# conix-center/pointcloud_stitching

Measured on AMD Instinct MI355X. Metric: Mpoints/s stitched (8x1280x720 streams: deproject+transform+RGB+pack), higher is better.
Workload: dtype f32

## Files before the change

pointcloud_stitching_amd/csrc/pcs_capi.cpp:

```cpp

#include <algorithm>
#include <cmath>
#include <cstdarg>
#include <cstdio>
#include <cstdlib>
#include <cstring>
#include <exception>
#include <new>
#include <string>
#include <vector>

#include "pcs_host.h"

using namespace pcs_host;

namespace pcs_host {

thread_local std::string g_create_err;

int fail(pcs_ctx* c, int status, const char* fmt, ...)
{
    char buf[512];
    va_list ap;
    va_start(ap, fmt);
// ... 133 lines not shown
bool certify_no_overflow(const pcs_stream_config& s, const Certificate& c, const float* M)
{
    if (!c.fast || !(c.p2_low > 0)) return false;
    if (s.color.model != PCS_DISTORTION_NONE && coeffs_nonzero(s.color)) return false;
    const double lim = std::ldexp(1.0, 30), infl = 1.0 + std::ldexp(1.0, -18);
    for (int r = 0; r < 3; r++) {
        double a = 0;
        for (int k = 0; k < 4; k++) if (!std::isfinite(M[4 * r + k])) return false;
        a = std::fabs((double)M[4 * r]) * c.xb + std::fabs((double)M[4 * r + 1]) * c.yb + std::fabs((double)M[4 * r + 2]) * c.zb +
            std::fabs((double)M[4 * r + 3]);
        if (!(a * 1000.0 * infl < lim)) return false;
    }
    const double x = c.a_max[0] / c.p2_low * infl, y = c.a_max[1] / c.p2_low * infl;
    const double xf = x * std::fabs((double)s.color.fx) * infl + std::fabs((double)s.color.ppx) + 2.0;
    const double yf = y * std::fabs((double)s.color.fy) * infl + std::fabs((double)s.color.ppy) + 2.0;
    return xf * infl < lim && yf * infl < lim;
}

bool row_magic(uint32_t W, uint32_t H, uint32_t& magic, uint32_t& shift)
{
    magic = shift = 0;
    if (W < 2) return false;
    uint32_t l = 0;
    while ((1ull << l) < W) l++;
    const unsigned __int128 m = (((unsigned __int128)1 << (31 + l)) / W) + 1;
    if (m >> 32) return false;
    magic = (uint32_t)m; shift = l - 1;
    auto ok = [&](uint64_t i) { return (uint32_t)(((uint64_t)i * magic) >> 32) >> shift == (uint32_t)(i / W); };
    for (uint64_t r = 0; r < H; r++) {
        const uint64_t a = r * W, b = r * W + W - 1;
        if (a >= (1ull << 31)) break;
        if (!ok(a) || (b < (1ull << 31) && !ok(b))) { magic = shift = 0; return false; }
    }
    if (!ok((1ull << 31) - 1)) { magic = shift = 0; return false; }
    return true;
}

uint32_t cutoff_dmax(const pcs_stream_config& s, const StreamParams& p, const std::vector<float>& mx)
{
    if (!p.z_zero_iff_d_zero || p.ddist || !(s.depth_scale > 0.0f)) return 0;
    double mxmax = 0;
    for (float v : mx) { if (!std::isfinite(v)) return 0; mxmax = std::max(mxmax, std::fabs((double)v)); }
    if (!(1.5 * mxmax < 2.0 - 1.0 / 1024.0)) return 0;
    const volatile float scale = s.depth_scale;
    auto z_of = [&](uint32_t d) { volatile float z = scale * (float)d; return (float)z; };
    if (!(z_of(1) > 0.0f)) return 0;
    for (uint32_t d = 1; d < 65535; d += 257) if (!(z_of(d) <= z_of(d + 1))) return 0;
    uint32_t lo = 0, hi = 65535;
    if (z_of(65535) <= 1.5f) return 65535;
    while (hi - lo > 1) { const uint32_t mid = (lo + hi) / 2; if (z_of(mid) <= 1.5f) lo = mid; else hi = mid; }
    return lo;
}

inline uint32_t tiles_of(uint32_t n) { return (n + kTilePoints - 1) / kTilePoints; }

int alloc_raster_slab(pcs_ctx* c, uint8_t*& slab, std::vector<uint16_t*>& depth, std::vector<uint8_t*>& color)
{
    const auto up = [](size_t b) { return (b + 16 + 255) & ~(size_t)255; };
    size_t total = 0;
    for (int s = 0; s < c->n_streams; s++)
        total += up((size_t)c->h_params[s].n_points * sizeof(uint16_t)) + up(c->h_params[s].color_bytes);
    void* q = nullptr;
    hipError_t e = hipMalloc(&q, total + 256);
    if (e != hipSuccess) return fail(c, PCS_ERR_NOMEM, "hipMalloc(%zu) failed: %s", total, hipGetErrorString(e));
    slab = static_cast<uint8_t*>(q);
    depth.assign(c->n_streams, nullptr); color.assign(c->n_streams, nullptr);
    size_t off = 0;
    for (int s = 0; s < c->n_streams; s++) {
        depth[s] = reinterpret_cast<uint16_t*>(slab + off);
        off += up((size_t)c->h_params[s].n_points * sizeof(uint16_t));
        color[s] = slab + off;
        off += up(c->h_params[s].color_bytes);
    }
    return PCS_OK;
}

int ensure_rasters(pcs_ctx* c)
{
    if (c->s_slab) return PCS_OK;
    return alloc_raster_slab(c, c->s_slab, c->s_depth, c->s_color);
}

}

namespace pcs_host {

int ensure_voxel_ws(pcs_ctx* c, size_t need)
{
    if (need <= c->s_voxel_ws_cap && c->s_voxel_ws) return PCS_OK;
    const size_t exact = need;
    if (c->s_voxel_ws) {
        HIPCHK(c, hipStreamSynchronize(c->stream));
        need += need / 4;
    }
    c->vox_state.clean = false;
    c->vox_state.spl_leaf = 0;
    int rc = ensure(c, c->s_voxel_ws, c->s_voxel_ws_cap, need);
    if (rc == PCS_ERR_NOMEM && need != exact) rc = ensure(c, c->s_voxel_ws, c->s_voxel_ws_cap, exact);
    return rc;
}

int acquire_event_pair(pcs_ctx* c, std::pair<hipEvent_t, hipEvent_t>& pr)
{
    if (!c->ev_free.empty()) { pr = c->ev_free.back(); c->ev_free.pop_back(); return PCS_OK; }
    HIPCHK(c, hipEventCreate(&pr.first));
    HIPCHK(c, hipEventCreate(&pr.second));
// ... 33 lines not shown
            HIPCHK(c, hipMemsetAsync(c->d_error, 0, sizeof(uint32_t), c->stream));
        }
        c->compact_seq++;
        if ((c->compact_seq & 0x3FFFFFFFu) == 0) {
            HIPCHK(c, hipMemsetAsync(c->d_desc, 0, sizeof(uint64_t) * ((size_t)c->total_tiles + PCS_MAX_STREAMS), c->stream));
            c->compact_seq++;
        }
        for (int s0 = 0; single_pass && s0 < c->n_streams; s0 += kLaunchStreams) {
            const int nl = std::min(kLaunchStreams, c->n_streams - s0);
            FramePtrs fp{};
            uint32_t tiles = 0;
            int m = 1;
            for (int k = 0; k < nl; k++) {
                fp.depth[k] = d_depth[s0 + k]; fp.color[k] = d_color[s0 + k];
                tiles += tiles_of(c->h_params[s0 + k].n_points);
                m = std::min(m, c->h_params[s0 + k].cert_fast);
            }
            CompactLaunch cl{};
            cl.d_ticket = c->compact_tickets ? c->d_ticket : nullptr; cl.ticket_base = c->tickets_issued;
            cl.d_desc = c->d_desc + c->h_params[s0].tile_base;
            cl.d_stream_end = c->d_stream_end;
            cl.d_stream_desc = c->d_desc + c->total_tiles;
            cl.d_chain_in = s0 > 0 ? c->d_stream_end + (s0 - 1) : nullptr;
            cl.d_error = c->d_error; cl.gen = c->compact_seq; cl.flags = c->flags;
            cl.d_counts = d_counts ? d_counts : c->d_counts; cl.n_total = c->n_streams;
            cl.last_launch = (s0 + nl == c->n_streams) ? 1 : 0;
            HIPCHK(c, launch_fused_compact(c->d_params, s0, nl, tiles, m >= 1 ? MathSel::Cert : MathSel::Ieee, fp, cl,
                                           d_payload, c->stream));
            c->tickets_issued += tiles;
        }
        if (c->kernel_timing) {
            HIPCHK(c, hipEventRecord(ev.second, c->stream));
            c->ev_pool.push_back(ev);
        }
        return PCS_OK;
    }
    if (pred) {
        for (int s0 = 0; !d_tile_kept && s0 < c->n_streams; s0 += kLaunchStreams) {
            const int nl = std::min(kLaunchStreams, c->n_streams - s0);
            FramePtrs fp{};
            uint32_t mp = 0;
            for (int k = 0; k < nl; k++) { fp.depth[k] = d_depth[s0 + k]; fp.color[k] = d_color[s0 + k]; mp = std::max(mp, c->h_params[s0 + k].n_points); }
            HIPCHK(c, launch_fused_count(c->d_params, s0, nl, mp, c->flags, fp, c->d_tile_counts, c->stream));
        }
        HIPCHK(c, launch_scan(c->d_params, c->n_streams, c->downsample, d_tile_kept ? d_tile_kept : c->d_tile_counts, c->d_tile_prefix,
                              c->d_stream_base, d_counts ? d_counts : c->d_counts, nullptr, c->stream));
    }
    for (int s0 = 0; s0 < c->n_streams; s0 += kLaunchStreams) {
        const int nl = std::min(kLaunchStreams, c->n_streams - s0);
        FramePtrs fp{};
        uint32_t mp = 0;
        for (int k = 0; k < nl; k++) { fp.depth[k] = d_depth[s0 + k]; fp.color[k] = d_color[s0 + k]; mp = std::max(mp, c->h_params[s0 + k].n_points); }
        bool fast = true, ident = true, noovf = true;
        bool dd = false, cd = false;
        for (int k = 0; k < nl; k++) {
            const StreamParams& q = c->h_params[s0 + k];
            fast &= q.cert_fast != 0; ident &= q.ident_r != 0; noovf &= q.no_overflow != 0;
            dd |= q.ddist != 0;
            cd |= q.cdist != 0 || q.tex_half != 0;
        }
        const MathSel sel = !fast ? MathSel::Ieee
                          : noovf ? (ident ? MathSel::CertIdentRNoOvf : MathSel::CertNoOvf)
                                  : (ident ? MathSel::CertIdentR : MathSel::Cert);
        if (dense)
            HIPCHK(c, launch_fused_dense(c->d_params, s0, nl, mp, dd, cd, sel, fp, d_payload, c->stream));
        else
            HIPCHK(c, launch_fused_emit(c->d_params, s0, nl, mp, c->flags, c->downsample, sel, fp, c->d_tile_prefix,
                                        c->d_stream_base, d_payload,
                                        pred ? (d_counts ? d_counts : c->d_counts) + c->n_streams : nullptr, c->n_streams, c->stream));
    }
    if (!pred && d_counts)
        HIPCHK(c, hipMemcpyAsync(d_counts, c->d_static_counts, sizeof(int32_t) * (c->n_streams + 1),
                                 hipMemcpyDeviceToDevice, c->stream));
    if (c->kernel_timing) {
        HIPCHK(c, hipEventRecord(ev.second, c->stream));
        c->ev_pool.push_back(ev);
    }
    return PCS_OK;
}

}

namespace {

int take_compact_error(pcs_ctx* c, bool& was_set)
{
    was_set = false;
    if (!c->d_error) return PCS_OK;
    uint32_t e = 0;
    HIPCHK(c, hipMemcpyAsync(&e, c->d_error, sizeof e, hipMemcpyDeviceToHost, c->stream));
    HIPCHK(c, hipStreamSynchronize(c->stream));
    if (e) {
        was_set = true;
        c->single_pass_ok = false;
        HIPCHK(c, hipMemsetAsync(c->d_error, 0, sizeof e, c->stream));
    }
    return PCS_OK;
}

int upload_params(pcs_ctx* c)
{
    HIPCHK(c, hipMemcpy(c->d_params, c->h_params.data(), c->h_params.size() * sizeof(StreamParams), hipMemcpyHostToDevice));
    return PCS_OK;
}

}

extern "C" {

int pcs_abi_version(void) { return PCS_ABI_VERSION; }

int pcs_device_count(void)
{
    int n = 0;
    hipError_t e = hipGetDeviceCount(&n);
    if (e != hipSuccess) return 0;
    return n;
}
// ... 144 lines not shown
            for (auto& pr : seen) if (pr.first == dim) { ok = pr.second; return hipSuccess; }
            hipError_t e;
            if (!d_bad && (e = hipMalloc((void**)&d_bad, sizeof(unsigned long long))) != hipSuccess) return e;
            if ((e = hipMemsetAsync(d_bad, 0, sizeof(unsigned long long), c->stream)) != hipSuccess) return e;
            const float cf = (float)dim, rc = (float)(1.0 / (double)cf);
            if ((e = launch_verify_div_const(cf, rc, dim, d_bad, c->stream)) != hipSuccess) return e;
            unsigned long long h = 1;
            if ((e = hipMemcpyAsync(&h, d_bad, sizeof h, hipMemcpyDeviceToHost, c->stream)) != hipSuccess) return e;
            if ((e = hipStreamSynchronize(c->stream)) != hipSuccess) return e;
            ok = (h == 0);
            seen.emplace_back(dim, ok);
            return hipSuccess;
        };
        for (int s = 0; s < c->n_streams; s++) {
            StreamParams& p = c->h_params[s];
            if (!p.cert_fast) continue;
            bool okw = false, okh = false;
            CREATE_CHK(verified(p.cW, okw));
            CREATE_CHK(verified(p.cH, okh));
            if (!(okw && okh)) { p.cert_fast = 0; p.ident_r = 0; p.no_overflow = 0; }
        }
        if (d_bad) (void)hipFree(d_bad);
    }
    c->compact_path = 0;
    if (const char* e = getenv("PCS_COMPACT_PATH")) {
        if (!strcmp(e, "single")) c->compact_path = 1;
    } else if (const char* e1 = getenv("PCS_COMPACT_SINGLE_PASS")) {
        if (e1[0] == '1') c->compact_path = 1;
    }
    c->single_pass_ok = c->compact_path == 1;
    { const char* e = getenv("PCS_COMPACT_TICKETS"); c->compact_tickets = e && e[0] == '1'; }
    c->math.resize(c->n_streams);
    for (int s = 0; s < c->n_streams; s++) {
        const StreamParams& q = c->h_params[s];
        c->math[s] = q.cert_fast ? ((q.ident_r ? 2 : 1) + (q.no_overflow ? 2 : 0)) : 0;
    }
    CREATE_CHK(hipMemcpy(c->d_params, c->h_params.data(), sizeof(StreamParams) * c->n_streams, hipMemcpyHostToDevice));
    {
        const char* env = getenv("PCS_ROW_CONST");
        const bool want = !(env && env[0] == '0');
        unsigned long long* d_bad = nullptr;
        bool any = false;
        for (int s = 0; want && s < c->n_streams; s++) {
            StreamParams& p = c->h_params[s];
            const float* t = c->cfg[s].depth_to_color.translation;
            if (p.ident_r != 1 || p.ddist || p.cdist || p.tex_half || t[1] != 0.0f || t[2] != 0.0f || !p.z_zero_iff_d_zero) continue;
            if (!d_bad) CREATE_CHK(hipMalloc((void**)&d_bad, sizeof(unsigned long long)));
            CREATE_CHK(hipMemsetAsync(d_bad, 0, sizeof(unsigned long long), c->stream));
            int32_t* d_crow = reinterpret_cast<int32_t*>(const_cast<float*>(p.my) + p.H);
            CREATE_CHK(launch_certify_color_row(c->d_params, s, p.H, d_crow, d_bad, c->stream));
            unsigned long long h = 1;
            CREATE_CHK(hipMemcpyAsync(&h, d_bad, sizeof h, hipMemcpyDeviceToHost, c->stream));
            CREATE_CHK(hipStreamSynchronize(c->stream));
            if (h == 0) { p.ident_r = 2; any = true; }
        }
        if (d_bad) (void)hipFree(d_bad);
        if (any) CREATE_CHK(hipMemcpy(c->d_params, c->h_params.data(), sizeof(StreamParams) * c->n_streams, hipMemcpyHostToDevice));
    }
#undef CREATE_CHK
    } catch (const std::exception& ex) {
        const int rc = fail(nullptr, PCS_ERR_NOMEM, "pcs_create: host allocation failed (%s)", ex.what());
        pcs_destroy(c);
        return rc;
    }
    *out = c;
    return PCS_OK;
}

void pcs_destroy(pcs_ctx* c)
{
    if (!c) return;
    DeviceGuard guard(c->device);
    if (c->stream) (void)hipStreamSynchronize(c->stream);
    for (float* p : c->d_lut) if (p) (void)hipFree(p);
    if (c->s_slab) (void)hipFree(c->s_slab);
    if (c->dl_stream) (void)hipStreamSynchronize(c->dl_stream);
    for (auto& sl : c->pipe) {
        if (sl.slab) (void)hipFree(sl.slab);
        if (sl.payload) (void)hipFree(sl.payload);
        if (sl.counts) (void)hipFree(sl.counts);
        if (sl.done) (void)hipEventDestroy(sl.done);
    }
    if (c->dl_stream) (void)hipStreamDestroy(c->dl_stream);
    void* singles[] = {c->d_params, c->d_tile_counts, c->d_tile_prefix, c->d_stream_base, c->d_counts, c->s_payload,
                       c->d_ticket, c->d_desc, c->d_stream_end, c->d_error, c->d_arrive, c->d_static_counts, c->d_batch_scratch, c->s_voxel_ws, c->s_voxel_in, c->s_voxel_out,
                       c->s_vertices, c->s_texcoords, c->s_pack_counts, c->s_pack_prefix};
    for (void* p : singles) if (p) (void)hipFree(p);
    for (auto& pr : c->ev_pool) { (void)hipEventDestroy(pr.first); (void)hipEventDestroy(pr.second); }
    for (auto& pr : c->ev_free) { (void)hipEventDestroy(pr.first); (void)hipEventDestroy(pr.second); }
    if (c->ev_begin) (void)hipEventDestroy(c->ev_begin);
    if (c->ev_end) (void)hipEventDestroy(c->ev_end);
    if (c->own_stream) (void)hipStreamDestroy(c->own_stream);
    delete c;
}

int pcs_set_cam_to_world(pcs_ctx* c, int stream, const float m16[16])
{
    if (!c || !m16) return PCS_ERR_INVALID_ARG;
    if (stream < 0 || stream >= c->n_streams) return fail(c, PCS_ERR_INVALID_ARG, "stream %d out of range", stream);
    DeviceGuard guard(c->device);
    HIPCHK(c, hipStreamSynchronize(c->stream));
    std::memcpy(c->cfg[stream].cam_to_world, m16, sizeof(float) * 16);
    StreamParams& q = c->h_params[stream];
    for (int k = 0; k < 12; k++) q.M[k] = m16[k];
    q.no_overflow = (q.cert_fast && certify_no_overflow(c->cfg[stream], c->cert[stream], m16)) ? 1 : 0;
    c->math[stream] = q.cert_fast ? ((q.ident_r ? 2 : 1) + (q.no_overflow ? 2 : 0)) : 0;
    return upload_params(c);
// ... 893 lines not shown
```

pointcloud_stitching_amd/csrc/pcs_device.h:

```cpp
#pragma once

#include <hip/hip_runtime.h>
#include <stdint.h>

#include "../../include/pcs_hip.h"

namespace pcs {

constexpr int      kBlockThreads   = 256;
constexpr int      kPointsPerLane  = 8;
constexpr uint32_t kTilePoints     = kBlockThreads * kPointsPerLane;
constexpr int      kLaunchStreams  = 16;

struct alignas(16) StreamParams {
    float    M[12];
    float    R[9];
    float    t[3];
    float    depth_scale;
    float    d_ppx, d_ppy, d_fx, d_fy;
    float    c_fx, c_fy, c_ppx, c_ppy;
    float    c_w_f, c_h_f;
    float    c_wm1_f, c_hm1_f;
    float    c_rw, c_rh;
    float    dk[5];
    float    ck[5];
    int32_t  W, H;
    int32_t  cW, cH;
    int32_t  bpp, stride;
    uint32_t color_bytes;
    uint32_t n_points;
    int32_t  ddist, cdist;
    uint32_t out_base;
    uint32_t tile_base;
    uint32_t w_magic, w_shift;
    int32_t  cert_fast;
    int32_t  ident_r;
    int32_t  no_overflow;
    int32_t  z_zero_iff_d_zero;
    uint32_t cut_dmax;
    int32_t  tex_half;
    const float* mx;
    const float* my;
};

struct FramePtrs {
    const uint16_t* depth[kLaunchStreams];
    const uint8_t*  color[kLaunchStreams];
};

struct VertexPtrs {
    const float*   vertices;
    const float*   texcoords;
    const uint8_t* color;
    uint32_t       n_points;
};

constexpr int kBatchEntries = 64;
constexpr int kBatchSets    = 16;
struct BatchPtrs {
    const uint16_t* depth[kBatchEntries];
    const uint8_t*  color[kBatchEntries];
    uint8_t*        payload[kBatchSets];
};
struct BatchCounts {
    int32_t* counts[kBatchSets];
};

constexpr int kPackBatch = 16;
struct PackBatch {
    VertexPtrs v[kPackBatch];
    uint8_t*   out[kPackBatch];
    int32_t    stream[kPackBatch];
};

enum class MathSel { Ieee = 0, Cert = 1, CertIdentR = 2, CertNoOvf = 3, CertIdentRNoOvf = 4,
                     CertRowConst = 5  };

hipError_t launch_fused_dense(const StreamParams* d_params, int stream0, int n_launch, uint32_t max_points,
                              bool any_ddist, bool any_cdist, MathSel math, const FramePtrs& fp, int16_t* d_payload,
                              hipStream_t st);

hipError_t launch_fused_count(const StreamParams* d_params, int stream0, int n_launch, uint32_t max_points,
                              uint32_t flags, const FramePtrs& fp, uint32_t* d_tile_counts, hipStream_t st);
hipError_t launch_scan(const StreamParams* d_params, int n_streams, int downsample,
                       const uint32_t* d_tile_counts, uint32_t* d_tile_prefix, uint32_t* d_stream_kept,
                       int32_t* d_counts, uint32_t* d_arrive, hipStream_t st);
hipError_t launch_fused_emit(const StreamParams* d_params, int stream0, int n_launch, uint32_t max_points,
                             uint32_t flags, int downsample, MathSel math, const FramePtrs& fp,
                             const uint32_t* d_tile_prefix, const uint32_t* d_stream_kept,
                             int16_t* d_payload, int32_t* d_total_out, int n_total_streams, hipStream_t st);
struct CompactLaunch {
    unsigned long long* d_ticket;
    unsigned long long  ticket_base;
    uint64_t*           d_desc;
    uint64_t*           d_stream_desc;
    uint32_t*           d_stream_end;
    const uint32_t*     d_chain_in;
    uint32_t*           d_error;
    uint32_t            gen;
    uint32_t            flags;
    int32_t*            d_counts;
    int32_t             n_total;
    int32_t             last_launch;
};
hipError_t launch_fused_compact(const StreamParams* d_params, int stream0, int n_launch, uint32_t launch_tiles,
                                MathSel math, const FramePtrs& fp, const CompactLaunch& cl, int16_t* d_payload,
                                hipStream_t st);

hipError_t launch_fused_dense_batch(const StreamParams* d_params, int n_streams, int n_sets, uint32_t max_points,
                                    bool any_ddist, bool any_cdist, MathSel math, const BatchPtrs& bp, hipStream_t st);
hipError_t launch_compact_batch(const StreamParams* d_params, int n_streams, int n_sets, uint32_t max_points,
                                uint32_t total_tiles, uint32_t flags, MathSel math, const BatchPtrs& bp,
                                const BatchCounts& bc, uint32_t* d_tile_counts, uint32_t* d_tile_prefix,
                                uint32_t* d_stream_kept, hipStream_t st);
hipError_t launch_verify_div_const(float c, float rc, int32_t dim, unsigned long long* d_bad, hipStream_t st);
hipError_t launch_certify_color_row(const StreamParams* d_params, int stream, int rows, int32_t* d_crow, unsigned long long* d_bad, hipStream_t st);

hipError_t launch_pack_dense(const StreamParams* d_params, int stream, const VertexPtrs& vp,
                             int16_t* d_out, hipStream_t st);
hipError_t launch_pack_count(const StreamParams* d_params, int stream, const VertexPtrs& vp, uint32_t flags,
                             uint32_t* d_tile_counts, hipStream_t st);
hipError_t launch_pack_scan(uint32_t n_tiles, const uint32_t* d_tile_counts, uint32_t* d_tile_prefix,
                            int32_t* d_out_points, uint32_t* d_arrive, hipStream_t st);
hipError_t launch_pack_emit(const StreamParams* d_params, int stream, const VertexPtrs& vp, uint32_t flags,
                            const uint32_t* d_tile_prefix, int16_t* d_out, hipStream_t st);

hipError_t launch_pack_batch(const StreamParams* d_params, const PackBatch& pb, int n, uint32_t max_points, bool aligned,
                             hipStream_t st);

// ... 67 lines not shown
```

pointcloud_stitching_amd/csrc/pcs_kernels.hip:

```cpp


#include <cstddef>

#include "pcs_device.h"

#ifndef PCS_TU_VOXEL
#define PCS_TU_VOXEL 0
#endif


#ifndef EMIT_WAVES
#define EMIT_WAVES 6
#endif

namespace pcs {

namespace {

constexpr uint32_t kDenseStageBytes = kTilePoints * PCS_POINT_BYTES;
constexpr uint32_t kStageBytes      = kTilePoints * PCS_POINT_BYTES + 32;

typedef float f32x4 __attribute__((ext_vector_type(4)));
template <class T> using gptr = const __attribute__((address_space(1))) T*;
template <class T> __device__ __forceinline__ gptr<T> as_global(const T* p)
// ... 93 lines not shown
    {
        q0 = __fdiv_rn(a0, b);
        q1 = __fdiv_rn(a1, b);
    }
    static __device__ __forceinline__ float div_const(float a, float c, float ) { return __fdiv_rn(a, c); }
};

template <bool IDENT_R, bool NO_OVERFLOW = false>
struct CertMath {
    static constexpr bool kIdentR = IDENT_R;
    static constexpr bool kRowConst = false;
    static constexpr int kCvtMode = NO_OVERFLOW ? 2 : 1;
    static __device__ __forceinline__ void d2c(const StreamParams& P, float X, float Y, float Z,
                                               float& P0, float& P1, float& P2)
    {
        if (IDENT_R) {
            P0 = __fadd_rn(X, P.t[0]);
            P1 = __fadd_rn(Y, P.t[1]);
            P2 = __fadd_rn(Z, P.t[2]);
        } else {
            IeeeMath::d2c(P, X, Y, Z, P0, P1, P2);
        }
    }
    static __device__ __forceinline__ void div2(float a0, float a1, float b, float& q0, float& q1)
    {
        float y = __builtin_amdgcn_rcpf(b);
        const float e = __fmaf_rn(-b, y, 1.0f);
        y = __fmaf_rn(e, y, y);
        float q = __fmul_rn(a0, y);
        float r = __fmaf_rn(-b, q, a0);
        q = __fmaf_rn(r, y, q);
        r = __fmaf_rn(-b, q, a0);
        q0 = __fmaf_rn(r, y, q);
        q = __fmul_rn(a1, y);
        r = __fmaf_rn(-b, q, a1);
        q = __fmaf_rn(r, y, q);
        r = __fmaf_rn(-b, q, a1);
        q1 = __fmaf_rn(r, y, q);
    }
    static __device__ __forceinline__ float div_const(float a, float c, float rc)
    {
        const float q0 = __fmul_rn(a, rc);
        const float r = __fmaf_rn(-c, q0, a);
        return __fmaf_rn(r, rc, q0);
    }
};

using CertNoOvf = CertMath<false, true>;
using CertIdentNoOvf = CertMath<true, true>;

struct CertRowConst : CertMath<true, false> {
    [[maybe_unused]] static constexpr bool kRowConst = true;
};

__device__ __forceinline__ void color_coords(const StreamParams& P, float u, float v, float& xf, float& yf)
{
    xf = __fmaf_rn(u, P.c_w_f, 0.5f);
    yf = __fmaf_rn(v, P.c_h_f, 0.5f);
}

template <class Cvt>
__device__ __forceinline__ uint32_t color_fetch(const StreamParams& P, const uint8_t* __restrict__ color,
                                                int32_t xi, int32_t yi, Cvt& cv)
{
    const uint32_t idx = __umul24((uint32_t)xi, (uint32_t)P.bpp) + __umul24((uint32_t)yi, (uint32_t)P.stride);
    uint32_t shift;
    const uint32_t off = cv.window(idx, P.color_bytes - 4u, shift);
    uint32_t w;
    __builtin_memcpy(&w, color + off, 4);
    return w >> shift;
}

__device__ __forceinline__ float world_mm(const float* __restrict__ Mr, float X, float Y, float Z)
{
    float a = __fmaf_rn(X, Mr[0], Mr[3]);
    a = __fmaf_rn(Y, Mr[1], a);
    a = __fmaf_rn(Z, Mr[2], a);
    return __fmul_rn(a, 1000.0f);
}

constexpr uint32_t kLoLo = 0x05040100u, kHiLo = 0x05040302u;
__device__ __forceinline__ uint32_t perm(uint32_t hi, uint32_t lo, uint32_t sel) { return __builtin_amdgcn_perm(hi, lo, sel); }

struct Record {
    uint32_t xy;
    uint32_t zc;
    uint32_t b;
};

__device__ __forceinline__ void stage_record(uint8_t* lds, uint32_t off, const Record& r)
{
    const bool odd = (off & 2u) != 0u;
    const uint32_t yz = perm(r.zc, r.xy, kHiLo);
    const uint32_t cc = perm(r.b, r.zc, kHiLo);
    const uint32_t h_val = odd ? r.xy : r.b;
    const uint32_t a_val = odd ? yz : r.xy;
    const uint32_t b_val = odd ? cc : r.zc;
    const uint32_t h_off = odd ? off : off + 8u;
    const uint32_t a_off = odd ? off + 2u : off;
    *reinterpret_cast<uint16_t*>(lds + h_off) = (uint16_t)h_val;
    *reinterpret_cast<uint32_t*>(lds + a_off) = a_val;
    *reinterpret_cast<uint32_t*>(lds + a_off + 4u) = b_val;
}

template <class Cvt>
__device__ __forceinline__ Record make_record(const StreamParams& P, const uint8_t* __restrict__ color,
// ... 310 lines not shown
__device__ __forceinline__ void store_staged(const uint8_t* lds, uint32_t head, uint32_t nbytes, uint8_t* g)
{
    uint8_t* g0 = g - head;
    const uint32_t end = head + nbytes;
    const uint32_t first_full = (head + 15u) >> 4;
    const uint32_t last_full = end >> 4;
    typedef uint32_t u32x4 __attribute__((ext_vector_type(4)));
    for (uint32_t j = first_full + threadIdx.x; j < last_full; j += THREADS)
        __builtin_nontemporal_store(reinterpret_cast<const u32x4*>(lds)[j], reinterpret_cast<u32x4*>(g0) + j);
    const uint32_t head_end = min(first_full << 4, end);
    for (uint32_t b = head + 2u * threadIdx.x; b < head_end; b += 2u * THREADS)
        *reinterpret_cast<uint16_t*>(g0 + b) = *reinterpret_cast<const uint16_t*>(lds + b);
    if (last_full >= first_full) {
        const uint32_t tail_begin = max(last_full << 4, head_end);
        for (uint32_t b = tail_begin + 2u * threadIdx.x; b < end; b += 2u * THREADS)
            *reinterpret_cast<uint16_t*>(g0 + b) = *reinterpret_cast<const uint16_t*>(lds + b);
    }
}

template <class Src, uint32_t THREADS = kBlockThreads>
__device__ __forceinline__ void dense_tile(const StreamParams& P, const Src& src, const uint8_t* __restrict__ color,
                                           uint32_t tile0, uint32_t n, uint8_t* __restrict__ out_bytes,
                                           uint4* stage)
{
    const uint32_t i0 = tile0 + threadIdx.x * kPointsPerLane;
    PointIn p[8];
    src.load8(P, i0, n, p);

    uint32_t w[20];
    auto fill = [&](auto& cv) {
#pragma unroll
        for (int k = 0; k < 8; k += 2) {
            const Record a = make_record(P, color, p[k], cv);
            const Record b = make_record(P, color, p[k + 1], cv);
            uint32_t* o = w + (k >> 1) * 5;
            o[0] = a.xy;
            o[1] = a.zc;
            o[2] = perm(b.xy, a.b, kLoLo);
            o[3] = perm(b.zc, b.xy, kHiLo);
            o[4] = perm(b.b, b.zc, kHiLo);
        }
    };
    if (Src::Math::kCvtMode == 2) {
        FastCvt<false> fast;
        fill(fast);
        if (__builtin_expect(fast.redo(), 0)) { ExactCvt exact; fill(exact); }
    } else if (Src::Math::kCvtMode == 1) {
        FastCvt<true> fast;
        fill(fast);
        if (__builtin_expect(fast.redo(), 0)) { ExactCvt exact; fill(exact); }
    } else {
        ExactCvt exact;
        fill(exact);
    }
    uint4* mine = stage + threadIdx.x * 5;
#pragma unroll
    for (int k = 0; k < 5; k++) mine[k] = make_uint4(w[4 * k], w[4 * k + 1], w[4 * k + 2], w[4 * k + 3]);
    __syncthreads();

    const uint32_t pts = min(THREADS * kPointsPerLane, n - tile0);
    store_staged<THREADS>(reinterpret_cast<const uint8_t*>(stage), 0u, pts * PCS_POINT_BYTES,
                          out_bytes + (size_t)tile0 * PCS_POINT_BYTES);
}

template <class Src, bool PRED, bool DS1>
__device__ __forceinline__ void generic_tile(const StreamParams& P, const Src& src, const uint8_t* __restrict__ color,
                                             uint32_t tile0, uint32_t n, uint32_t flags, uint32_t ds,
                                             uint32_t g0, uint32_t out_first, uint8_t* __restrict__ payload_bytes,
                                             uint8_t* stage, uint32_t* wsum)
{
    if (DS1) ds = 1u;
    const uint32_t i0 = tile0 + threadIdx.x * kPointsPerLane;
    PointIn p[8];
    src.load8(P, i0, n, p);

    uint32_t keep, ex = 0;
    if (PRED) {
        keep = keep_mask8(p, i0, n, flags);
        uint32_t wave_total;
        ex = wave_exclusive_scan(__popc(keep), wave_total);
        if ((threadIdx.x & 63) == 63) wsum[threadIdx.x >> 6] = wave_total;
    } else {
        const uint32_t mine = (i0 < n) ? min(8u, n - i0) : 0u;
        keep = (1u << mine) - 1u;
    }

    Record rec[8];
    auto fill = [&](auto& cv) {
#pragma unroll
        for (int k = 0; k < 8; k++) rec[k] = make_record(P, color, p[k], cv);
    };
    if (Src::Math::kCvtMode == 2) {
        FastCvt<false> fast;
        fill(fast);
        if (__builtin_expect(fast.redo(), 0)) { ExactCvt exact; fill(exact); }
    } else if (Src::Math::kCvtMode == 1) {
        FastCvt<true> fast;
        fill(fast);
        if (__builtin_expect(fast.redo(), 0)) { ExactCvt exact; fill(exact); }
    } else {
        ExactCvt exact;
        fill(exact);
    }

    uint32_t lane_first, tile_kept;
    if (PRED) {
// ... 161 lines not shown

    uint8_t* gdst = payload_bytes + (size_t)q_lo * PCS_POINT_BYTES;
    const uint32_t head = (uint32_t)((uintptr_t)gdst & 15u);
    uint32_t rank = lane_first;
#pragma unroll
    for (int k = 0; k < 8; k++) {
        if ((keep >> k) & 1u) {
            stage_record(stage, head + rank * PCS_POINT_BYTES, rec[k]);
            rank++;
        }
    }
    __syncthreads();
    store_staged(stage, head, tile_kept * PCS_POINT_BYTES, gdst);
}

#endif

template <bool LEAN = false, bool IDENT_R = false>
__device__ __forceinline__ void request_constants(const StreamParams& P, const void* a, const void* b, const void* c = nullptr)
{
    static_assert(sizeof(StreamParams) == 19 * 16, "request_constants covers the struct in 19 quads");
    static_assert(offsetof(StreamParams, dk) == 39 * 4 && offsetof(StreamParams, ck) == 44 * 4 && offsetof(StreamParams, R) == 12 * 4,
                  "quads 10, 11 = dk[1..4], ck[0..3]; quads 3, 4 = R[0..7]");
    typedef uint32_t u32x4s __attribute__((ext_vector_type(4)));
    const u32x4s* q = reinterpret_cast<const u32x4s*>(&P);
    if (LEAN && IDENT_R)
        asm volatile("" :: "s"(q[0]), "s"(q[1]), "s"(q[2]), "s"(q[5]), "s"(q[6]), "s"(q[7]), "s"(q[8]), "s"(q[9]),
                           "s"(q[12]), "s"(q[13]), "s"(q[14]), "s"(q[15]), "s"(q[16]), "s"(q[17]), "s"(q[18]),
                           "s"(a), "s"(b), "s"(c));
    else if (LEAN)
        asm volatile("" :: "s"(q[0]), "s"(q[1]), "s"(q[2]), "s"(q[3]), "s"(q[4]), "s"(q[5]), "s"(q[6]), "s"(q[7]), "s"(q[8]), "s"(q[9]),
                           "s"(q[12]), "s"(q[13]), "s"(q[14]), "s"(q[15]), "s"(q[16]), "s"(q[17]), "s"(q[18]),
                           "s"(a), "s"(b), "s"(c));
    else
        asm volatile("" :: "s"(q[0]), "s"(q[1]), "s"(q[2]), "s"(q[3]), "s"(q[4]), "s"(q[5]), "s"(q[6]), "s"(q[7]), "s"(q[8]), "s"(q[9]),
                           "s"(q[10]), "s"(q[11]), "s"(q[12]), "s"(q[13]), "s"(q[14]), "s"(q[15]), "s"(q[16]), "s"(q[17]), "s"(q[18]),
                           "s"(a), "s"(b), "s"(c));
}

#if !PCS_TU_VOXEL

template <bool DDIST, bool CDIST, class Mth, uint32_t THREADS = kBlockThreads>
__global__ __launch_bounds__(THREADS, 7)
void pcs_fused_dense_kernel(const StreamParams* __restrict__ params, int stream0, FramePtrs fp,
                            uint8_t* __restrict__ payload_bytes)
{
    __shared__ uint4 stage[THREADS * kPointsPerLane * PCS_POINT_BYTES / 16];
    const int s = blockIdx.y;
    const StreamParams& P = params[stream0 + s];
    request_constants(P, fp.depth[s], fp.color[s], payload_bytes);
    const uint32_t n = P.n_points;
    const uint32_t tile0 = blockIdx.x * (THREADS * kPointsPerLane);
    if (tile0 >= n) return;
    DepthSource<DDIST, CDIST, Mth> src{fp.depth[s]};
    dense_tile<DepthSource<DDIST, CDIST, Mth>, THREADS>(P, src, fp.color[s], tile0, n, payload_bytes + (size_t)P.out_base * PCS_POINT_BYTES, stage);
}

template <bool DDIST, bool CDIST, class Mth>
__global__ __launch_bounds__(kBlockThreads, 7)
void pcs_fused_dense_batch_kernel(const StreamParams* __restrict__ params, BatchPtrs bp)
{
    __shared__ uint4 stage[kDenseStageBytes / 16];
    const int s = blockIdx.y;
    const StreamParams& P = params[s];
    const int e = blockIdx.z * gridDim.y + s;
    request_constants(P, bp.depth[e], bp.color[e], bp.payload[blockIdx.z]);
    const uint32_t n = P.n_points;
    const uint32_t tile0 = blockIdx.x * kTilePoints;
    if (tile0 >= n) return;
    DepthSource<DDIST, CDIST, Mth> src{bp.depth[e]};
    dense_tile(P, src, bp.color[e], tile0, n, bp.payload[blockIdx.z] + (size_t)P.out_base * PCS_POINT_BYTES, stage);
}

constexpr int kCountTiles = 2;
template <bool DDIST, bool CDIST>
__device__ __forceinline__ void count_tiles(const StreamParams& P, const uint16_t* __restrict__ dp, uint32_t flags,
                                            uint32_t* __restrict__ tile_counts, uint32_t (*wsum)[4])
{
    const uint32_t n = P.n_points;
    const uint32_t tile_first = blockIdx.x * kCountTiles;
    if (tile_first * kTilePoints >= n) return;
    uint32_t c[kCountTiles];
    const bool cut = (flags & PCS_FLAG_CUTOFF) != 0;
    if (P.z_zero_iff_d_zero && (!cut || P.cut_dmax != 0u)) {
        const uint32_t dmax = cut ? P.cut_dmax : 0xFFFFu;
        uint4 dv[kCountTiles];
        const bool aligned = ((uintptr_t)dp & 15) == 0 && n >= 8;
        if (aligned) {
#pragma unroll
            for (int q = 0; q < kCountTiles; q++) {
                const uint32_t i0 = (tile_first + q) * kTilePoints + threadIdx.x * kPointsPerLane;
                dv[q] = *reinterpret_cast<const uint4*>(dp + ((i0 + 8 <= n) ? i0 : 0u));
            }
        } else {
#pragma unroll
            for (int q = 0; q < kCountTiles; q++) dv[q] = make_uint4(0, 0, 0, 0);
        }
#pragma unroll
        for (int q = 0; q < kCountTiles; q++) {
            const uint32_t i0 = (tile_first + q) * kTilePoints + threadIdx.x * kPointsPerLane;
            uint32_t dw[4] = {dv[q].x, dv[q].y, dv[q].z, dv[q].w};
            if (!(aligned && i0 + 8 <= n)) {
                dw[0] = dw[1] = dw[2] = dw[3] = 0u;
                for (uint32_t k = 0; k < 8 && i0 + k < n; k++) dw[k >> 1] |= (uint32_t)dp[i0 + k] << ((k & 1u) * 16u);
            }
            uint32_t rng = 0, nz = 0;
#pragma unroll
            for (int k = 0; k < 8; k++) {
// ... 938 lines not shown
    uint32_t local = 0;
    for (uint32_t d = 1u + threadIdx.x; d < 65536u; d += 256u) local += row_of(d) != want;
    if (local) atomicAdd(bad, (unsigned long long)local);
    if (threadIdx.x == 0) crow[r] = want;
}


__global__ __launch_bounds__(256)
void pcs_verify_div_const_kernel(float c, float rc, int32_t dim, unsigned long long* __restrict__ bad)
{
    const uint64_t stride = (uint64_t)gridDim.x * blockDim.x;
    uint32_t local = 0;
    for (uint64_t bits = (uint64_t)blockIdx.x * blockDim.x + threadIdx.x; bits < (1ull << 32); bits += stride) {
        const float a = __uint_as_float((uint32_t)bits);
        const float f1 = __fmaf_rn(IeeeMath::div_const(a, c, rc), c, 0.5f);
        const float f2 = __fmaf_rn(CertMath<false>::div_const(a, c, rc), c, 0.5f);
        const int32_t i1 = min(max(cvtt_x86(f1), 0), dim - 1);
        const int32_t i2 = min(max(cvtt_x86(f2), 0), dim - 1);
        const int32_t i3 = (f2 >= 2147483648.0f) ? i2 : min(max(cvt_sat(f2), 0), dim - 1);
        local += (i1 != i2) | (i2 != i3);
    }
    if (local) atomicAdd(bad, (unsigned long long)local);
}

#endif

constexpr uint32_t kSmallThreads = 64, kSmallTilePoints = kSmallThreads * kPointsPerLane;
inline bool small_launch(uint32_t, int)
{
    const char* v = getenv("PCS_SMALL_TILES");
    return v && v[0] == '1';
}

inline dim3 tile_grid(uint32_t max_points, int n_launch)
{
    return dim3((max_points + kTilePoints - 1) / kTilePoints, (unsigned)n_launch, 1);
}

}


#if !PCS_TU_VOXEL
hipError_t launch_fused_dense(const StreamParams* d_params, int stream0, int n_launch, uint32_t max_points,
                              bool any_ddist, bool any_cdist, MathSel math, const FramePtrs& fp, int16_t* d_payload,
                              hipStream_t st)
{
    if (n_launch <= 0 || max_points == 0) return hipSuccess;
    const bool small = small_launch(max_points, n_launch);
    const dim3 grid = small ? dim3((max_points + kSmallTilePoints - 1) / kSmallTilePoints, (unsigned)n_launch, 1) : tile_grid(max_points, n_launch);
#define L(DD, CD, M) do { if (small) hipLaunchKernelGGL((pcs_fused_dense_kernel<DD, CD, M, kSmallThreads>), grid, dim3(kSmallThreads), 0, st, \
                                        d_params, stream0, fp, reinterpret_cast<uint8_t*>(d_payload)); \
                          else hipLaunchKernelGGL((pcs_fused_dense_kernel<DD, CD, M>), grid, dim3(kBlockThreads), 0, st, \
                                        d_params, stream0, fp, reinterpret_cast<uint8_t*>(d_payload)); } while (0)
    if (math != MathSel::Ieee && !any_ddist) {
        const bool ident = (math == MathSel::CertIdentR || math == MathSel::CertIdentRNoOvf);
        const bool noovf = (math == MathSel::CertNoOvf || math == MathSel::CertIdentRNoOvf) && !any_cdist;
        if (noovf)      { if (ident) L(false, false, CertIdentNoOvf); else L(false, false, CertNoOvf); }
        else if (ident) { if (any_cdist) L(false, true, CertMath<true>); else L(false, false, CertMath<true>); }
        else            { if (any_cdist) L(false, true, CertMath<false>); else L(false, false, CertMath<false>); }
    } else {
        if (any_ddist) { if (any_cdist) L(true, true, IeeeMath); else L(true, false, IeeeMath); }
        else           { if (any_cdist) L(false, true, IeeeMath); else L(false, false, IeeeMath); }
    }
#undef L
    return hipGetLastError();
}

hipError_t launch_fused_count(const StreamParams* d_params, int stream0, int n_launch, uint32_t max_points,
                              uint32_t flags, const FramePtrs& fp, uint32_t* d_tile_counts, hipStream_t st)
{
    if (n_launch <= 0 || max_points == 0) return hipSuccess;
    const uint32_t tiles = (max_points + kTilePoints - 1) / kTilePoints;
    const dim3 grid((tiles + kCountTiles - 1) / kCountTiles, (unsigned)n_launch, 1);
    hipLaunchKernelGGL((pcs_fused_count_kernel<true, false>), grid, dim3(kBlockThreads), 0, st,
                       d_params, stream0, fp, flags, d_tile_counts);
    return hipGetLastError();
}

hipError_t launch_scan(const StreamParams* d_params, int n_streams, int downsample,
                       const uint32_t* d_tile_counts, uint32_t* d_tile_prefix, uint32_t* d_stream_kept,
                       int32_t* d_counts, uint32_t* d_arrive, hipStream_t st)
{
    hipLaunchKernelGGL(pcs_scan_kernel, dim3((unsigned)n_streams), dim3(1024), 0, st, d_params, 0, n_streams, 0u,
                       (uint32_t)downsample, d_tile_counts, d_tile_prefix, d_stream_kept, d_counts, d_arrive);
    return hipGetLastError();
}

hipError_t launch_fused_emit(const StreamParams* d_params, int stream0, int n_launch, uint32_t max_points,
                             uint32_t flags, int downsample, MathSel math, const FramePtrs& fp,
                             const uint32_t* d_tile_prefix, const uint32_t* d_stream_kept,
                             int16_t* d_payload, int32_t* d_total_out, int n_total_streams, hipStream_t st)
{
    if (n_launch <= 0 || max_points == 0) return hipSuccess;
    const dim3 grid = tile_grid(max_points, n_launch);
    const bool pred = (flags & (PCS_FLAG_CUTOFF | PCS_FLAG_DROP_INVALID)) != 0;
    const bool ds1 = downsample == 1;
    uint8_t* out = reinterpret_cast<uint8_t*>(d_payload);
#define L(PR, D1, M) hipLaunchKernelGGL((pcs_fused_emit_kernel<PR, D1, M>), grid, dim3(kBlockThreads), 0, st, d_params, \
                                        stream0, fp, flags, (uint32_t)downsample, d_tile_prefix, d_stream_kept, out, \
                                        d_total_out, n_total_streams)
#define LM(M) do { if (pred) { if (ds1) L(true, true, M); else L(true, false, M); } \
                   else      { if (ds1) L(false, true, M); else L(false, false, M); } } while (0)
    const bool ident = (math == MathSel::CertIdentR || math == MathSel::CertIdentRNoOvf);
    if (math == MathSel::Ieee) LM(IeeeMath); else if (ident) LM(CertMath<true>); else LM(CertMath<false>);
#undef LM
#undef L
// ... 234 lines not shown
```

Measured before the change: 319,300.

## Stage per-wave color row windows into LDS for row-constant dense kernel

Adds a specialized dense kernel path for streams certified to have row-constant color rows and no overflow. Each wave computes the span of color bytes its points can reach, prefetches that window into LDS with global_load_lds_dwordx4, then gathers RGB from LDS instead of scattered global loads, falling back to global reads for misses. Window bounds are precomputed on the host at create time and stored after the color row table. The path uses inline asm with hand-placed waitcnts and requires 16-byte-aligned buffers, which adds fragility in exchange for removing uncoalesced color gathers.

After: 334,100 (median of 6 runs). +4.6%, better.

```diff
diff --git a/pointcloud_stitching_amd/csrc/pcs_capi.cpp b/pointcloud_stitching_amd/csrc/pcs_capi.cpp
--- a/pointcloud_stitching_amd/csrc/pcs_capi.cpp
+++ b/pointcloud_stitching_amd/csrc/pcs_capi.cpp
@@ -209,6 +209,21 @@
     return lo;
 }
 
+constexpr double kWinShiftCols = 48.0;
+void color_window_params(const StreamParams& p, float tx, int32_t out[3])
+{
+    const double a = (double)p.c_fx / p.d_fx, b = (double)p.c_ppx - (double)p.d_ppx * a + 0.5;
+    const double room = ((3072.0 - 2 * 34) / p.bpp - 512.0 * a) / 2.0 - 4.0;
+    const double shift = std::max(0.0, std::min(kWinShiftCols, room));
+    const double lo = b - 2.0 - (tx < 0.0f ? shift : 0.0), hi = b + 2.0 + (tx > 0.0f ? shift : 0.0);
+    const double kx = std::round(a * 4096.0);
+    const double reach = kx * p.W + 4096.0 * std::max(std::fabs(lo), std::fabs(hi)) + 4096.0;
+    if (!(a > 0.0) || !(reach < 2147483647.0)) { out[0] = 0; out[1] = 0; out[2] = -4096; return; }
+    out[0] = (int32_t)kx;
+    out[1] = (int32_t)std::floor(lo * 4096.0);
+    out[2] = (int32_t)std::ceil(hi * 4096.0);
+}
+
 inline uint32_t tiles_of(uint32_t n) { return (n + kTilePoints - 1) / kTilePoints; }
 
 int alloc_raster_slab(pcs_ctx* c, uint8_t*& slab, std::vector<uint16_t*>& depth, std::vector<uint8_t*>& color)
@@ -348,10 +363,12 @@
         uint32_t mp = 0;
         for (int k = 0; k < nl; k++) { fp.depth[k] = d_depth[s0 + k]; fp.color[k] = d_color[s0 + k]; mp = std::max(mp, c->h_params[s0 + k].n_points); }
         bool fast = true, ident = true, noovf = true;
+        bool rowc = true;
         bool dd = false, cd = false;
         for (int k = 0; k < nl; k++) {
             const StreamParams& q = c->h_params[s0 + k];
             fast &= q.cert_fast != 0; ident &= q.ident_r != 0; noovf &= q.no_overflow != 0;
+            rowc &= q.ident_r == 2 && (q.W & 7) == 0 && q.color_bytes >= 16;
             dd |= q.ddist != 0;
             cd |= q.cdist != 0 || q.tex_half != 0;
         }
@@ -359,7 +376,8 @@
                           : noovf ? (ident ? MathSel::CertIdentRNoOvf : MathSel::CertNoOvf)
                                   : (ident ? MathSel::CertIdentR : MathSel::Cert);
         if (dense)
-            HIPCHK(c, launch_fused_dense(c->d_params, s0, nl, mp, dd, cd, sel, fp, d_payload, c->stream));
+            HIPCHK(c, launch_fused_dense(c->d_params, s0, nl, mp, dd, cd, sel == MathSel::CertIdentRNoOvf && rowc ? MathSel::CertRowConstNoOvf : sel,
+                                         fp, d_payload, c->stream));
         else
             HIPCHK(c, launch_fused_emit(c->d_params, s0, nl, mp, c->flags, c->downsample, sel, fp, c->d_tile_prefix,
                                         c->d_stream_base, d_payload,
@@ -610,7 +628,12 @@
             unsigned long long h = 1;
             CREATE_CHK(hipMemcpyAsync(&h, d_bad, sizeof h, hipMemcpyDeviceToHost, c->stream));
             CREATE_CHK(hipStreamSynchronize(c->stream));
-            if (h == 0) { p.ident_r = 2; any = true; }
+            if (h == 0) {
+                p.ident_r = 2; any = true;
+                int32_t win[3];
+                color_window_params(p, t[0], win);
+                CREATE_CHK(hipMemcpy(d_crow + p.H, win, sizeof win, hipMemcpyHostToDevice));
+            }
         }
         if (d_bad) (void)hipFree(d_bad);
         if (any) CREATE_CHK(hipMemcpy(c->d_params, c->h_params.data(), sizeof(StreamParams) * c->n_streams, hipMemcpyHostToDevice));
diff --git a/pointcloud_stitching_amd/csrc/pcs_device.h b/pointcloud_stitching_amd/csrc/pcs_device.h
--- a/pointcloud_stitching_amd/csrc/pcs_device.h
+++ b/pointcloud_stitching_amd/csrc/pcs_device.h
@@ -74,7 +74,8 @@
 };
 
 enum class MathSel { Ieee = 0, Cert = 1, CertIdentR = 2, CertNoOvf = 3, CertIdentRNoOvf = 4,
-                     CertRowConst = 5  };
+                     CertRowConst = 5 ,
+                     CertRowConstNoOvf = 6  };
 
 hipError_t launch_fused_dense(const StreamParams* d_params, int stream0, int n_launch, uint32_t max_points,
                               bool any_ddist, bool any_cdist, MathSel math, const FramePtrs& fp, int16_t* d_payload,
diff --git a/pointcloud_stitching_amd/csrc/pcs_kernels.hip b/pointcloud_stitching_amd/csrc/pcs_kernels.hip
--- a/pointcloud_stitching_amd/csrc/pcs_kernels.hip
+++ b/pointcloud_stitching_amd/csrc/pcs_kernels.hip
@@ -169,6 +169,9 @@
 struct CertRowConst : CertMath<true, false> {
     [[maybe_unused]] static constexpr bool kRowConst = true;
 };
+struct CertRowConstNoOvf : CertMath<true, true> {
+    [[maybe_unused]] static constexpr bool kRowConst = true;
+};
 
 __device__ __forceinline__ void color_coords(const StreamParams& P, float u, float v, float& xf, float& yf)
 {
@@ -585,6 +588,159 @@
     } else {
         ExactCvt exact;
         fill(exact);
+    }
+    uint4* mine = stage + threadIdx.x * 5;
+#pragma unroll
+    for (int k = 0; k < 5; k++) mine[k] = make_uint4(w[4 * k], w[4 * k + 1], w[4 * k + 2], w[4 * k + 3]);
+    __syncthreads();
+
+    const uint32_t pts = min(THREADS * kPointsPerLane, n - tile0);
+    store_staged<THREADS>(reinterpret_cast<const uint8_t*>(stage), 0u, pts * PCS_POINT_BYTES,
+                          out_bytes + (size_t)tile0 * PCS_POINT_BYTES);
+}
+
+constexpr uint32_t kWaveStageBytes = 64u * kPointsPerLane * PCS_POINT_BYTES;
+constexpr uint32_t kWinPieces      = 3;
+constexpr uint32_t kWinBytes       = kWinPieces * 64u * 16u;
+constexpr uint32_t kWinZeroWord    = kWaveStageBytes - 16u;
+static_assert(kWinBytes + 8u <= kWinZeroWord, "the windows, the dword read past their end and the zero word fit one wave's stage");
+
+template <class T> using cptr = const __attribute__((address_space(4))) T*;
+
+__device__ __forceinline__ void color_stretch(const StreamParams& P, const int32_t (&wp)[3], int32_t crow, int32_t c0, int32_t c1,
+                                              uint32_t room, uint32_t& ws, uint32_t& len)
+{
+    const int32_t lo = min(max((c0 * wp[0] + wp[1]) >> 12, 0), P.cW - 1);
+    const int32_t hi = min(max((c1 * wp[0] + wp[2]) >> 12, 0), P.cW - 1);
+    const uint32_t row = (uint32_t)crow * (uint32_t)P.stride;
+    ws = (row + (uint32_t)lo * (uint32_t)P.bpp) & ~15u;
+    const uint32_t we = min((row + (uint32_t)hi * (uint32_t)P.bpp + 4u + 15u) & ~15u, P.color_bytes & ~15u);
+    len = min(we > ws ? we - ws : 0u, room);
+}
+
+typedef uint32_t u32x4v __attribute__((ext_vector_type(4)));
+__device__ __forceinline__ u32x4v load16_asm(const void* base, uint32_t off)
+{
+    u32x4v v;
+    asm volatile("global_load_dwordx4 %0, %1, %2" : "=v"(v) : "v"(off), "s"(base));
+    return v;
+}
+__device__ __forceinline__ uint32_t load4_asm(const void* base, uint32_t off)
+{
+    uint32_t v;
+    asm volatile("global_load_dword %0, %1, %2" : "=v"(v) : "v"(off), "s"(base));
+    return v;
+}
+__device__ __forceinline__ void window_piece(const uint8_t* color, uint32_t off, uint32_t lds)
+{
+    uint32_t keep;
+    asm volatile("s_mov_b32 %0, m0\n\ts_mov_b32 m0, %3\n\ts_nop 0\n\tglobal_load_lds_dwordx4 %1, %2\n\ts_mov_b32 m0, %0"
+                 : "=&s"(keep) : "v"(off), "s"(color), "s"(lds) : "memory");
+}
+
+template <class Mth, uint32_t THREADS = kBlockThreads>
+__device__ __forceinline__ void dense_tile_rowc(const StreamParams& P, const uint16_t* __restrict__ depth,
+                                                const uint8_t* __restrict__ color, uint32_t tile0, uint32_t n,
+                                                uint8_t* __restrict__ out_bytes, uint4* stage)
+{
+    static_assert(Mth::kRowConst && Mth::kCvtMode == 2, "the no-overflow row-constant policy");
+    const uint32_t i0 = tile0 + threadIdx.x * kPointsPerLane;
+    const uint32_t ic = min(i0, n - kPointsPerLane);
+    const uint32_t r = P.w_magic ? (__umulhi(ic, P.w_magic) >> P.w_shift) : ic / (uint32_t)P.W;
+    const uint32_t c0 = ic - r * (uint32_t)P.W;
+    u32x4v dv = load16_asm(depth, ic * 2u);
+    u32x4v ma = load16_asm(P.mx, c0 * 4u);
+    u32x4v mb = load16_asm(P.mx, c0 * 4u + 16u);
+    uint32_t myb = load4_asm(P.my, r * 4u);
+    uint32_t crow = load4_asm(P.my, ((uint32_t)P.H + r) * 4u);
+
+    const uint32_t wave = __builtin_amdgcn_readfirstlane(threadIdx.x >> 6);
+    const uint32_t iw = tile0 + wave * 64u * kPointsPerLane;
+    const uint32_t il = min(iw + 64u * kPointsPerLane, n) - 1u;
+    const uint32_t ra = __builtin_amdgcn_readfirstlane(r), rb = __builtin_amdgcn_readlane(r, 63);
+    const cptr<int32_t> tab = (cptr<int32_t>)(uintptr_t)(P.my + P.H);
+    const int32_t wp[3] = {tab[P.H], tab[P.H + 1], tab[P.H + 2]};
+    const uint32_t lrel = wave * kWaveStageBytes;
+    uint32_t wsa = 0, lena = 0, wsb = 0, lenb = 0;
+    if (iw < n) {
+        color_stretch(P, wp, tab[ra], (int32_t)(iw - ra * (uint32_t)P.W), ra == rb ? (int32_t)(il - ra * (uint32_t)P.W) : P.W - 1,
+                      kWinBytes, wsa, lena);
+        if (rb != ra) color_stretch(P, wp, tab[rb], 0, (int32_t)(il - rb * (uint32_t)P.W), kWinBytes - lena, wsb, lenb);
+    }
+    const uint32_t lane = threadIdx.x & 63u;
+    const uint32_t pieces = max((lena + lenb) >> 4, 1u), pa = lena >> 4;
+    const uint32_t lds0 = (uint32_t)(uintptr_t)(__attribute__((address_space(3))) uint8_t*)stage + lrel;
+#pragma unroll
+    for (uint32_t k = 0; k < kWinPieces; k++) {
+        const uint32_t j = min(k * 64u + lane, pieces - 1u);
+        window_piece(color, j < pa ? wsa + 16u * j : wsb + 16u * (j - pa), lds0 + k * 1024u);
+    }
+    if (lane == 0) *reinterpret_cast<uint32_t*>(reinterpret_cast<uint8_t*>(stage) + lrel + kWinZeroWord) = *(cptr<uint32_t>)(uintptr_t)color;
+
+    static_assert(kWinPieces == 3, "the wait below leaves the window's requests in flight");
+    asm volatile("s_waitcnt vmcnt(3)" : "+v"(dv), "+v"(ma), "+v"(mb), "+v"(myb), "+v"(crow));
+    PointIn p[8];
+    {
+        const uint32_t dw[4] = {dv.x, dv.y, dv.z, dv.w};
+        const uint32_t mxs[8] = {ma.x, ma.y, ma.z, ma.w, mb.x, mb.y, mb.z, mb.w};
+#pragma unroll
+        for (int k = 0; k < 8; k++) {
+            const uint32_t d = (k & 1) ? (dw[k >> 1] >> 16) : (dw[k >> 1] & 0xFFFFu);
+            p[k] = deproject_pixel_rowc<Mth>(P, d, __uint_as_float(mxs[k]), __uint_as_float(myb), (int)crow);
+        }
+    }
+    FastCvt<false> cv;
+    uint32_t xy[8], zz[8], ci[8];
+#pragma unroll
+    for (int k = 0; k < 8; k++) {
+        const float ax = world_mm(P.M + 0, p[k].X, p[k].Y, p[k].Z);
+        const float ay = world_mm(P.M + 4, p[k].X, p[k].Y, p[k].Z);
+        const float az = world_mm(P.M + 8, p[k].X, p[k].Y, p[k].Z);
+        xy[k] = perm((uint32_t)cv.cvt(ay), (uint32_t)cv.cvt(ax), kLoLo);
+        zz[k] = (uint32_t)cv.cvt(az);
+        const int32_t xi = cv.pixel(__fmaf_rn(p[k].u, P.c_w_f, 0.5f), P.cW - 1, P.c_wm1_f);
+        ci[k] = __umul24((uint32_t)xi, (uint32_t)P.bpp) + __umul24((uint32_t)__float_as_int(p[k].v), (uint32_t)P.stride);
+    }
+    const bool in_a = r == ra;
+    const uint32_t ws = in_a ? wsa : wsb, len = in_a ? lena : lenb;
+    const uint32_t wn = len > 3u ? len - 3u : 0u;
+    const uint32_t lb = lrel + (in_a ? 0u : lena), lz = lrel + kWinZeroWord;
+    asm volatile("s_waitcnt vmcnt(0)" : "+v"(ci[0]), "+v"(ci[1]), "+v"(ci[2]), "+v"(ci[3]), "+v"(ci[4]), "+v"(ci[5]), "+v"(ci[6]),
+                 "+v"(ci[7]) :: "memory");
+    uint32_t wc[8];
+    bool miss = false;
+#pragma unroll
+    for (int k = 0; k < 8; k++) {
+        const uint32_t o = ci[k] - ws;
+        const bool in = o < wn;
+        const uint32_t* qa = reinterpret_cast<const uint32_t*>(reinterpret_cast<const uint8_t*>(stage) + (in ? (lb + o) & ~3u : lz));
+        wc[k] = __builtin_amdgcn_alignbyte(qa[1], qa[0], ci[k]);
+        miss |= !in && ci[k] != 0u;
+    }
+    if (__builtin_expect(miss, 0)) {
+#pragma unroll
+        for (int k = 0; k < 8; k++) {
+            if (!(ci[k] - ws < wn) && ci[k] != 0u) {
+                ExactCvt exact;
+                uint32_t shift;
+                const uint32_t off = exact.window(ci[k], P.color_bytes - 4u, shift);
+                uint32_t g;
+                __builtin_memcpy(&g, color + off, 4);
+                wc[k] = g >> shift;
+            }
+        }
+    }
+    uint32_t w[20];
+#pragma unroll
+    for (int k = 0; k < 8; k += 2) {
+        const Record a{xy[k], perm(wc[k], zz[k], kLoLo), __builtin_amdgcn_ubfe(wc[k], 16, 8)};
+        const Record b{xy[k + 1], perm(wc[k + 1], zz[k + 1], kLoLo), __builtin_amdgcn_ubfe(wc[k + 1], 16, 8)};
+        uint32_t* o = w + (k >> 1) * 5;
+        o[0] = a.xy;
+        o[1] = a.zc;
+        o[2] = perm(b.xy, a.b, kLoLo);
+        o[3] = perm(b.zc, b.xy, kHiLo);
+        o[4] = perm(b.b, b.zc, kHiLo);
     }
     uint4* mine = stage + threadIdx.x * 5;
 #pragma unroll
@@ -852,8 +1008,12 @@
     const uint32_t n = P.n_points;
     const uint32_t tile0 = blockIdx.x * (THREADS * kPointsPerLane);
     if (tile0 >= n) return;
-    DepthSource<DDIST, CDIST, Mth> src{fp.depth[s]};
-    dense_tile<DepthSource<DDIST, CDIST, Mth>, THREADS>(P, src, fp.color[s], tile0, n, payload_bytes + (size_t)P.out_base * PCS_POINT_BYTES, stage);
+    if constexpr (Mth::kRowConst) {
+        dense_tile_rowc<Mth, THREADS>(P, fp.depth[s], fp.color[s], tile0, n, payload_bytes + (size_t)P.out_base * PCS_POINT_BYTES, stage);
+    } else {
+        DepthSource<DDIST, CDIST, Mth> src{fp.depth[s]};
+        dense_tile<DepthSource<DDIST, CDIST, Mth>, THREADS>(P, src, fp.color[s], tile0, n, payload_bytes + (size_t)P.out_base * PCS_POINT_BYTES, stage);
+    }
 }
 
 template <bool DDIST, bool CDIST, class Mth>
@@ -1898,6 +2058,12 @@
                                         d_params, stream0, fp, reinterpret_cast<uint8_t*>(d_payload)); \
                           else hipLaunchKernelGGL((pcs_fused_dense_kernel<DD, CD, M>), grid, dim3(kBlockThreads), 0, st, \
                                         d_params, stream0, fp, reinterpret_cast<uint8_t*>(d_payload)); } while (0)
+    if (math == MathSel::CertRowConstNoOvf) {
+        bool aligned = !any_ddist && !any_cdist;
+        for (int k = 0; k < n_launch; k++) aligned &= ((((uintptr_t)fp.color[k]) | ((uintptr_t)fp.depth[k])) & 15u) == 0;
+        if (aligned) { L(false, false, CertRowConstNoOvf); return hipGetLastError(); }
+        math = MathSel::CertIdentRNoOvf;
+    }
     if (math != MathSel::Ieee && !any_ddist) {
         const bool ident = (math == MathSel::CertIdentR || math == MathSel::CertIdentRNoOvf);
         const bool noovf = (math == MathSel::CertNoOvf || math == MathSel::CertIdentRNoOvf) && !any_cdist;
```
